# nipponjo/tts-arabic-pytorch

Hardware: AMD Instinct MI355X
Metric: audio samples/sec (FastPitch+HiFi-GAN, synthetic 64-phoneme inputs) (higher is better)
Workload: dtype f32

## Files before the change

tts-arabic-pytorch_amd/csrc/api.hip:

```cpp
#include <cerrno>
#include <cstdio>
#include <cstdlib>
#include <cstring>
#include <algorithm>
#include <atomic>
#include <mutex>
#include <string>
#include <vector>

#include "kernels.hpp"

namespace ttsamd {

static thread_local std::string g_err;

void set_error(const char* fmt, ...) {
    char buf[1024];
    va_list ap;
    va_start(ap, fmt);
    vsnprintf(buf, sizeof(buf), fmt, ap);
    va_end(ap);
    g_err = buf;
}

// ... 905 lines not shown
    float* wino = nullptr;
    if (default_precision() == 0 && convt_wino_packable(cin, cout, u) && opt_int(OPT_CONVT_WINO, 1) != 0) {
        wino = packed + 2 * n;
        const int64_t nw = (int64_t)(6 * cin + 1) * u * cout;
        hipLaunchKernelGGL(pack_convt_wino_kernel, dim3((unsigned)((nw + 255) / 256)), dim3(256), 0, s, w, bias, cin, cout, u, wino);
        TTS_CHECK_HIP(hipGetLastError());
    }
    ConvParams p;
    std::memset(&p, 0, sizeof(p));
    p.batch = batch;
    p.lens_in = lens; p.lens_out = lens;
    prof_begin(s, 2.0 * cout * cin * 2 * u);
    const int32_t rc = launch_upsampler(p, x, packed, planes, bias, y, cin, cout, u, 2 * u, lin, 1, in_slope, opt_int(OPT_CONVT, 1) != 0, s, wino,
                                        wino ? wino + (int64_t)6 * cin * u * cout : nullptr);
    prof_end(s);
    return rc;
}

int64_t ttsamd_resblock_pair_packed_floats(int32_t channels, int32_t k, int32_t variant) {
    if (channels < 1 || k < 1) return 0;
    const int64_t n = 2 * (int64_t)channels * k * channels;
    const int nwino = (variant == 4 ? 1 : (variant == 5 ? 2 : 0));
    if (variant == 6) return n + ((k == 3 || k == 7 || k == 11) ? 2 * (int64_t)channels * wino4_groups(k) * channels : 0);
    return n + ((k == 3 || k == 7 || k == 11) ? nwino * (int64_t)channels * wino2_groups(k) * channels : 0);
}

int32_t ttsamd_resblock_pair(const float* x, float* y, const float* w1, const float* b1, const float* w2, const float* b2,
                             int32_t channels, int32_t k, int32_t dil, const int64_t* lens, int32_t len_mul, int32_t L,
                             int32_t batch, int32_t mode, float div, float slope, int32_t variant, float* packed, int64_t packed_floats,
                             void* stream) {
    TTS_REQUIRE(x && y && w1 && b1 && w2 && b2 && packed && channels % 32 == 0 && k >= 1 && batch >= 1 && L >= 1 && len_mul >= 1 &&
                mode >= 0 && mode <= 2, "resblock_pair: bad argument");
    TTS_REQUIRE(packed_floats >= ttsamd_resblock_pair_packed_floats(channels, k, variant),
                "resblock_pair: `packed` holds %lld floats, variant %d at C = %d, k = %d needs %lld (ttsamd_resblock_pair_packed_floats)",
                (long long)packed_floats, variant, channels, k, (long long)ttsamd_resblock_pair_packed_floats(channels, k, variant));
    hipStream_t s = (hipStream_t)stream;
    const int64_t n = (int64_t)channels * k * channels;
    for (int i = 0; i < 2; ++i) {
        hipLaunchKernelGGL(pack_conv_weight_kernel, dim3((unsigned)((n + 255) / 256)), dim3(256), 0, s, i == 0 ? w1 : w2, channels,
                           channels, k, channels, packed + i * n);
        TTS_CHECK_HIP(hipGetLastError());
    }
    const double fl = 2.0 * (2.0 * channels * channels * k);
    int32_t rc;
    prof_begin(s, fl);
    if (variant == 1) {
// ... 4 lines not shown
            TTS_REQUIRE((k == 3 || k == 7 || k == 11) && (channels <= 64 || (variant == 5 && channels == 128)),
                        "resblock_pair: variants 4 / 5 are built for C = 32 / 64 (5: and 128), k = 3 / 7 / 11");
            const int64_t nw = (int64_t)channels * wino2_groups(k) * channels;
            for (int i = 0; i < (variant == 5 ? 2 : 1); ++i) {
                float* wino = packed + 2 * n + i * nw;
                hipLaunchKernelGGL(pack_wino2_weight_kernel, dim3((unsigned)((nw + 255) / 256)), dim3(256), 0, s, i == 0 ? w2 : w1, channels,
                                   channels, k, channels, wino);
                TTS_CHECK_HIP(hipGetLastError());
                (i == 0 ? w2w : w1w) = wino;
            }
        }
        rc = launch_fused_pair2(channels, x, y, packed, b1, packed + n, b2, k, dil, lens, len_mul, L, batch, mode, div, slope,
                                variant == 3 ? 1 : 2, s, w2w, w1w);
    } else if (variant == 6) {
        TTS_REQUIRE(channels == 32 && (k == 3 || k == 7 || k == 11), "resblock_pair: variant 6 is built for C = 32, k = 3 / 7 / 11");
        const int64_t nw4 = (int64_t)channels * wino4_groups(k) * channels;
        for (int i = 0; i < 2; ++i) {
            hipLaunchKernelGGL(pack_wino4_weight_kernel, dim3((unsigned)((nw4 + 255) / 256)), dim3(256), 0, s, i == 0 ? w1 : w2, channels,
                               channels, k, channels, packed + 2 * n + i * nw4);
            TTS_CHECK_HIP(hipGetLastError());
        }
        rc = launch_fused_pair4(channels, x, y, packed + 2 * n, b1, packed + 2 * n + nw4, b2, k, dil, lens, len_mul, L, batch, mode, div,
                                slope, s);
    } else if (variant == -1) {
        rc = 0;
    } else {
        set_error("resblock_pair: variant %d (1: first generation, 2 / 3: second generation with 256- / 128-column blocks, 4 / 5: 256 columns + Winograd phase B / both phases, 6: C = 32 with both phases on Winograd F(4,3))", variant);
        rc = TTSAMD_EINVAL;
    }
    prof_end(s);
    return rc;
}

int64_t ttsamd_resblock2_packed_floats(int32_t channels, int32_t k, int32_t variant) {
    if (channels < 1 || k < 1 || (variant != 1 && variant != 2)) return 0;
    return 2 * (int64_t)channels * k * channels;
}

int32_t ttsamd_resblock2(const float* x, float* y, const float* w1, const float* b1, const float* w2, const float* b2, int32_t channels,
                         int32_t k, int32_t dil1, int32_t dil2, const int64_t* lens, int32_t len_mul, int32_t L, int32_t batch, int32_t mode,
                         float div, float slope, int32_t variant, float* packed, int64_t packed_floats, void* stream) {
    TTS_REQUIRE(x && y && w1 && b1 && w2 && b2 && packed && channels % 32 == 0 && channels >= 32 && k >= 1 && batch >= 1 && L >= 1 &&
                len_mul >= 1 && mode >= 0 && mode <= 2 && x != y, "resblock2: bad argument");
    TTS_REQUIRE(variant == 1 || variant == 2, "resblock2: variant %d (1: two single-conv launches, 2: both convs in one launch)", variant);
    TTS_REQUIRE(packed_floats >= ttsamd_resblock2_packed_floats(channels, k, variant),
                "resblock2: `packed` holds %lld floats, C = %d, k = %d needs %lld (ttsamd_resblock2_packed_floats)", (long long)packed_floats,
                channels, k, (long long)ttsamd_resblock2_packed_floats(channels, k, variant));
    if (variant == 1) {
        TTS_REQUIRE(resblock2_conv_supported(channels, k, dil1, L, x, y) && resblock2_conv_supported(channels, k, dil2, L, x, y),
                    "resblock2: variant 1 does not cover C = %d, k = %d, dilations %d / %d (C = 32 / 64 / 128, k = 3 / 5 / 7 / 11, "
// ... 80 lines not shown
```

tts-arabic-pytorch_amd/csrc/common.hpp:

```cpp
#pragma once
#include <hip/hip_runtime.h>
#include <stdint.h>
#include <atomic>
#include <cstdarg>
#include <cstdio>
#include <cstdlib>
#include <string>

#include "../../include/ttsamd.h"

namespace ttsamd {

void set_error(const char* fmt, ...);

#define TTS_CHECK_HIP(expr)                                                         \
    do {                                                                            \
        hipError_t e_ = (expr);                                                     \
        if (e_ != hipSuccess) {                                                     \
            ttsamd::set_error("%s failed: %s (%s:%d)", #expr, hipGetErrorString(e_), \
                              __FILE__, __LINE__);                                  \
            return TTSAMD_EHIP;                                                     \
        }                                                                           \
    } while (0)

// ... 13 lines not shown

inline int64_t align_up(int64_t x, int64_t a) { return (x + a - 1) / a * a; }

inline hipError_t lds_opt_in(const void* fn, int bytes, std::atomic<uint64_t>& done) {
    int dev = 0;
    hipError_t e = hipGetDevice(&dev);
    if (e != hipSuccess) return e;
    if (dev >= 0 && dev < 64 && ((done.load(std::memory_order_acquire) >> dev) & 1)) return hipSuccess;
    e = hipFuncSetAttribute(fn, hipFuncAttributeMaxDynamicSharedMemorySize, bytes);
    if (e == hipSuccess && dev >= 0 && dev < 64) done.fetch_or(1ull << dev, std::memory_order_release);
    return e;
}

#define TTS_OPTIONS(X)                                                                                     \
    X(HIFIGAN_STREAMS, 0, 0, 1)    \
    X(WINO, 0, 0, 1)                                              \
    X(WINO2, 0, 0, 31)             \
    X(WINO4, 0, 0, 127)            \
    X(FUSED_PAIR, 0, 0, 1)                   \
    X(FUSED2, 0, 0, 1)                                           \
    X(FUSED2_MASK, 1, 0, 0x1ff)               \
    X(FUSED2_MASK_N1, 1, 0, 0x1ff)          \
    X(FUSED2_WB, 0, 0, 2)                     \
    X(PAIR4, 0, 0, 1)              \
    X(CONVT, 0, 0, 1)                              \
    X(CONVT_WINO, 0, 0, 2)         \
    X(BFO, 0, 0, 1)                \
    X(BFO_CHAIN, 0, 0, 1)                           \
    X(BFO_CHAIN7, 0, 0, 1)                                 \
    X(BFO_FF, 0, 0, 1)                              \
    X(BFO_SPLITK, 0, 0, 1)                                              \
    X(BFO_SMALL_TILES, 0, 0, 1)            \
    X(BF16_ATTN, 0, 0, 1)                                         \
    X(BF16_PACKED_T, 0, 0, 1)                   \
    X(ATT_RA, 0, 1, 4)                             \
    X(ATT_SPLIT, 0, 0, 1)                      \
    X(XCD_W, 0, 0, 1)                            \
    X(XCD_WMAX_KB, 0, 0, 1 << 20)     \
    X(DEEP_SPLITK, 0, 0, 1)        \
    X(TACO_PERSISTENT, 0, 0, 2)    \
    X(TACO_SEG, 0, 8, 1 << 20)     \
    X(RESBLOCK2_PAIR, 1, 0, 0x3f)
enum Opt : int {
#define TTS_OPT_ENUM(name, kind, lo, hi) OPT_##name,
    TTS_OPTIONS(TTS_OPT_ENUM)
#undef TTS_OPT_ENUM
    OPT_COUNT
// ... 68 lines not shown
void note_conv_launch(int32_t route, int32_t ksplit);
void last_conv_launch(int32_t* route, int32_t* ksplit);
bool convt_supported(const ConvParams& p);
int32_t launch_convt(const ConvParams& p, hipStream_t stream);
int32_t launch_upsampler(ConvParams& p, const float* x, const float* w, const void* w_bf16, const float* bias, float* y, int cin, int cout,
                         int u, int kt, int L, int len_mul, float in_slope, bool convt_ok, hipStream_t stream, const float* w_wino = nullptr,
                         const float* bias_wino = nullptr);
bool convt_wino_packable(int cin, int cout, int u);
void pack_convt_wino_weight(const float* w, const float* bias, int cin, int cout, int u, float* out_w, float* out_bias);
bool convt_wino_supported(const ConvParams& p, const float* w_wino, const float* bias_wino);
int32_t launch_convt_wino(const ConvParams& p, const float* w_wino, const float* bias_wino, hipStream_t stream);
bool fused_pair_supported(int32_t channels, int32_t k, int32_t dil, int32_t L, const float* x, const float* y);
int32_t launch_fused_pair(int32_t channels, const float* x, float* y, const float* w1, const float* b1, const float* w2,
                          const float* b2, int32_t k, int32_t dil, const int64_t* lens, int32_t len_mul, int32_t L, int32_t batch,
                          int32_t mode, float div, float slope, hipStream_t stream);
bool fused_pair2_supported(int32_t channels, int32_t k, int32_t dil, int32_t L, const float* x, const float* y, int32_t ntw);
int32_t launch_fused_pair2(int32_t channels, const float* x, float* y, const float* w1, const float* b1, const float* w2,
                           const float* b2, int32_t k, int32_t dil, const int64_t* lens, int32_t len_mul, int32_t L, int32_t batch,
                           int32_t mode, float div, float slope, int32_t ntw, hipStream_t stream, const float* w2_wino = nullptr,
                           const float* w1_wino = nullptr);
bool fused_pair4_supported(int32_t channels, int32_t k, int32_t dil, int32_t L, const float* x, const float* y);
int32_t launch_fused_pair4(int32_t channels, const float* x, float* y, const float* w1_wino4, const float* b1, const float* w2_wino4,
                           const float* b2, int32_t k, int32_t dil, const int64_t* lens, int32_t len_mul, int32_t L, int32_t batch,
                           int32_t mode, float div, float slope, hipStream_t stream);
bool resblock2_conv_supported(int32_t channels, int32_t k, int32_t dil, int32_t L, const float* x, const float* y);
int32_t launch_resblock2_conv(int32_t channels, const float* x, float* y, const float* w, const float* b, int32_t k, int32_t dil,
                              const int64_t* lens, int32_t len_mul, int32_t L, int32_t batch, int32_t mode, float div, float slope,
                              hipStream_t stream);
bool resblock2_pair_supported(int32_t channels, int32_t k, int32_t d1, int32_t d2, int32_t L, const float* x, const float* y);
int32_t launch_resblock2_pair(int32_t channels, const float* x, float* y, const float* w1, const float* b1, const float* w2,
                              const float* b2, int32_t k, int32_t d1, int32_t d2, const int64_t* lens, int32_t len_mul, int32_t L,
                              int32_t batch, int32_t mode, float div, float slope, hipStream_t stream);
int wino_route(const ConvParams& p);
int32_t launch_wino(const ConvParams& p, hipStream_t stream);
void pack_wino_weight(const float* w, int cout, int cin, float* out);
int wino2_groups(int k);
int wino2_block_outputs(int coutp, int dil);
int32_t launch_wino2(const ConvParams& p, hipStream_t stream);
void pack_wino2_weight(const float* w, int cout, int cin, int k, float* out);
int wino4_groups(int k);
int wino44_groups(int k);
constexpr int kWino4Default = 127;
bool wino44_wanted(const ConvParams& p);
int wino4_block_outputs(int dil);
int wino4_ksplit(const ConvParams& p);
int32_t launch_splitk_reduce(const ConvParams& q, hipStream_t stream);
int32_t launch_wino4(const ConvParams& p, hipStream_t stream);
// ... 48 lines not shown
```

tts-arabic-pytorch_amd/csrc/hifigan.hip:

```cpp
#include <cmath>
#include <cstring>
#include <cstdlib>
#include <map>
#include <mutex>
#include <string>
#include <vector>

#include "kernels.hpp"
#include "bfo.hpp"

namespace ttsamd {

constexpr unsigned kFused2Mask = 0x00F;
constexpr int kPair4MinK = 7;
constexpr unsigned kFused2MaskN1 = 0x000;
constexpr int64_t kFused2SmallColumns = 2 * 256 * 252;

constexpr unsigned kResblock2PairMask = 0x00;

static bool resblock2_pair_choice(unsigned mask, int32_t channels, int32_t k, int32_t d1, int32_t d2, int32_t L, const float* x,
                                  const float* y) {
    const int ci = channels == 32 ? 0 : (channels == 64 ? 1 : -1);
    const int ki = k == 3 ? 0 : (k == 5 ? 1 : (k == 7 ? 2 : -1));
    if (ci < 0 || ki < 0 || !(mask & (1u << (3 * ci + ki)))) return false;
    return resblock2_pair_supported(channels, k, d1, d2, L, x, y);
}

struct ConvW {
    int64_t w_off = 0, b_off = 0;
    int64_t w16_off = 0, w_n = 0;
    BfoWeightOffs wo;
    int64_t ww44_off = -1;
    int64_t ww4_off = -1;
    int64_t wct_off = -1, bct_off = -1;
    int64_t ww_off = -1;
    int cin = 0, cout = 0, k = 0;
};
// ... 9 lines not shown
    int hop = 1;
    bool rb2 = false;
    int64_t max_cl = 0;
    bool bfo_ok = false;
    mutable std::mutex mu;
    mutable hipStream_t side[2] = {nullptr, nullptr};
    mutable hipEvent_t ev_fork = nullptr, ev_done[3] = {nullptr, nullptr, nullptr};
};

static bool use_branch_streams(const HifiGan* h, int32_t B, int32_t T) {
    if (h->cfg.n_kernels != 3) return false;
    const int64_t streams = opt_int(OPT_HIFIGAN_STREAMS, -1);
    if (streams >= 0) return streams == 1;
    if (default_precision() == 1 && h->bfo_ok) {
        if (opt_int(OPT_BFO, 1) != 0) return (int64_t)B * T >= 8192;
    }
    return true;
}

struct Fused2Switches {
    bool on = true, mask_forced = false;
    bool wino_b = true, wino_a = true;
    bool pair4 = true;
    unsigned mask = kFused2Mask, mask_n1 = kFused2MaskN1;
};
static Fused2Switches read_fused2_switches() {
    Fused2Switches sw;
    sw.on = opt_int(OPT_FUSED2, 1) != 0;
    const int64_t m = opt_int(OPT_FUSED2_MASK, -1);
    sw.mask_forced = m >= 0;
    if (sw.mask_forced) sw.mask = (unsigned)m;
    sw.mask_n1 = (unsigned)opt_int(OPT_FUSED2_MASK_N1, kFused2MaskN1);
    const int64_t wb = opt_int(OPT_FUSED2_WB, 2);
    sw.wino_b = wb != 0;
    sw.wino_a = wb == 2;
    sw.pair4 = opt_int(OPT_PAIR4, 1) != 0;
    return sw;
}

static int fused2_choice(const Fused2Switches& sw, int32_t channels, int32_t k, int32_t dil, int32_t L, const float* x, const float* y,
                         int64_t columns) {
    if (!sw.on) return 0;
    const int ci = channels == 32 ? 0 : (channels == 64 ? 1 : (channels == 128 ? 2 : -1));
    const int ki = k == 3 ? 0 : (k == 7 ? 1 : (k == 11 ? 2 : -1));
    if (ci < 0 || ki < 0) return 0;
    const unsigned bit = 1u << (3 * ci + ki);
    const bool small = columns < (int64_t)kFused2SmallColumns && !sw.mask_forced;
    if (small) return 0;
    if (!(sw.mask & bit)) return 0;
    int ntw = (sw.mask_n1 & bit) ? 1 : 2;
    if (!fused_pair2_supported(channels, k, dil, L, x, y, ntw)) {
        ntw = 3 - ntw;
        if (!fused_pair2_supported(channels, k, dil, L, x, y, ntw)) return 0;
    }
    return ntw;
}

using TensorMap = std::map<std::string, const ttsamd_tensor*>;

// ... 66 lines not shown
    TTS_TRY(folded_weight(tm, base, 3, w, shp));
    TTS_REQUIRE(shp[0] == cout && shp[1] == cin && shp[2] == k, "hifigan: '%s' has shape [%lld,%lld,%lld], expected [%d,%d,%d]",
                base.c_str(), (long long)shp[0], (long long)shp[1], (long long)shp[2], cout, cin, k);
    cw.cin = cin; cw.cout = cout; cw.k = k;
    cw.w_off = (int64_t)blob.size();
    blob.resize(blob.size() + (size_t)cin * k * cout_padded(cout));
    pack_conv_weight(w.data(), cout, cin, k, blob.data() + cw.w_off);
    if (direct_only) {
        blob.resize(align_up((int64_t)blob.size(), 64));
        return get_bias(tm, base, cout, blob, cw.b_off);
    }
    add_bf16(blob, blob16, cw, (int64_t)cin * k * cout_padded(cout));
    if ((k == 3 || k == 7 || k == 11) && cin % 8 == 0 && cout % 32 == 0) {
        blob.resize(align_up((int64_t)blob.size(), 64));
        cw.ww_off = (int64_t)blob.size();
        blob.resize(blob.size() + (size_t)cin * wino2_groups(k) * cout_padded(cout));
        pack_wino2_weight(w.data(), cout, cin, k, blob.data() + cw.ww_off);
        if (cout >= 64 || (cout == 32 && cin == 32 && k >= kPair4MinK)) {
            blob.resize(align_up((int64_t)blob.size(), 64));
            cw.ww4_off = (int64_t)blob.size();
            blob.resize(blob.size() + (size_t)cin * wino4_groups(k) * cout_padded(cout));
            pack_wino4_weight(w.data(), cout, cin, k, blob.data() + cw.ww4_off);
        }
        if (cout >= 64 && wino44_groups(k) != 0) {
            blob.resize(align_up((int64_t)blob.size(), 64));
            cw.ww44_off = (int64_t)blob.size();
            blob.resize(blob.size() + (size_t)cin * wino44_groups(k) * cout_padded(cout));
            pack_wino44_weight(w.data(), cout, cin, k, blob.data() + cw.ww44_off);
        }
    }
    if (cin % 8 == 0 && cout % 32 == 0) cw.wo = bfo_append_weights(w.data(), cout, cin, k, 1, blob16);
    blob.resize(align_up((int64_t)blob.size(), 64));
    return get_bias(tm, base, cout, blob, cw.b_off);
}

void hifigan_destroy(HifiGan* h);

__global__ void hifigan_touch_kernel() {}

int32_t hifigan_create(const ttsamd_tensor* weights, int32_t n, const ttsamd_hifigan_cfg* cfg, HifiGan** out) {
    TTS_REQUIRE(weights && cfg && out, "hifigan_create: null argument");
    TTS_REQUIRE(cfg->n_ups >= 1 && cfg->n_ups <= 8 && cfg->n_kernels >= 1 && cfg->n_kernels <= 8 &&
                cfg->n_dilations >= 1 && cfg->n_dilations <= 8, "hifigan_create: bad config counts");
    const int rb = cfg->resblock == 0 ? 1 : cfg->resblock;
    TTS_REQUIRE(rb == 1 || rb == 2, "hifigan_create: resblock %d (1 = ResBlock1, 2 = ResBlock2)", cfg->resblock);
    TTS_REQUIRE(rb == 1 || cfg->n_dilations >= 2, "hifigan_create: a ResBlock2 takes two dilations per kernel size, %d given",
                cfg->n_dilations);
// ... 203 lines not shown
    } join{false, bs[1], bs[2]};
    const auto fail = [&](int32_t rc) { join.on = multi && rc != 0; return rc; };

    ConvParams p;
    std::memset(&p, 0, sizeof(p));
    p.batch = B;
    p.lens_in = lens; p.lens_out = lens;
    p.n_phase = 1; p.div = 1.f;
    p.splitk_ws = splitks[0]; p.splitk_floats = kSplitKFloats;
    const bool pack_t = default_precision() == 1 && opt_int(OPT_BF16_PACKED_T, 1) != 0;
    const Fused2Switches f2sw = read_fused2_switches();
    const bool fused_ok = default_precision() == 0 && opt_int(OPT_FUSED_PAIR, 1) != 0;
    const bool convt_ok = opt_int(OPT_CONVT, 1) != 0;
    const unsigned rb2_mask = (unsigned)opt_int(OPT_RESBLOCK2_PAIR, kResblock2PairMask);
    bool in_section = false;
    int pack_io = 0;
    auto conv = [&](const ConvW& cw, const float* x, hipStream_t st, float* y, const float* res, int L, int mul,
                    int dil, float slope, int mode, float div) -> int32_t {
        p.x = x; p.x_bs = (int64_t)cw.cin * L; p.x_cs = L;
        p.w = h->dev + cw.w_off; p.bias = h->dev + cw.b_off;
        p.w_bf16 = h->dev16 + cw.w16_off; p.precision = default_precision();
        p.w_wino = cw.ww_off >= 0 ? h->dev + cw.ww_off : nullptr;
        p.w_wino4 = (cw.ww4_off >= 0 && cw.cout >= 64) ? h->dev + cw.ww4_off : nullptr;
        p.w_wino44 = cw.ww44_off >= 0 ? h->dev + cw.ww44_off : nullptr;
        p.y = y; p.y_bs = (int64_t)cw.cout * L; p.y_cs = L; p.y_ts = 1;
        p.res = res; p.r_bs = (int64_t)cw.cout * L; p.r_cs = L;
        p.len_in_mul = mul; p.len_out_mul = mul; p.Lin = L; p.Nout = L;
        p.Cin = cw.cin; p.Cout = cw.cout; p.CoutP = cout_padded(cw.cout); p.K = cw.k;
        p.dil = dil; p.pad = (cw.k * dil - dil) / 2;
        p.n_phase = 1; p.phase_p = 0;
        p.in_slope = slope; p.relu_out = 0; p.mode = mode; p.div = div;
        p.x_packed = (pack_io & 1) ? 1 : 0; p.y_packed = (pack_io & 2) ? 1 : 0; p.pack_slope = 0.1f;
        if (in_section) prof_add(2.0 * cw.cout * cw.cin * cw.k * mul);
        else prof_begin(st, 2.0 * cw.cout * cw.cin * cw.k * mul);
        const int32_t rc = launch_conv(p, st);
        if (!in_section) prof_end(st);
        return rc;
    };

#define HG_TRY(expr) do { int32_t rc_ = (expr); if (rc_ != 0) return fail(rc_); } while (0)
#define HG_CHECK_HIP(expr) do { hipError_t e_ = (expr); if (e_ != hipSuccess) { set_error("%s failed: %s (%s:%d)", #expr, hipGetErrorString(e_), __FILE__, __LINE__); return fail(TTSAMD_EHIP); } } while (0)
    const int prec = default_precision();
    if ((prec == 1 || prec == 2) && h->bfo_ok && opt_int(OPT_BFO, 1) != 0) {
        const BfoMode& M = bfo_mode(prec);
        const uint16_t* W16 = h->dev16;
        void *curo = cur, *upso = ups_out;
        HG_TRY(M.pack(mel, B, cfg.num_mels, T, 1.f, mel_o, s));
// ... 155 lines not shown
                                            0.1f, st);
                if (!in_section) prof_end(st);
                HG_TRY(rc2);
            }
            if (multi) HG_CHECK_HIP(hipEventRecord(h->ev_done[j], st));
        }
        for (int j = 0; !h->rb2 && j < cfg.n_kernels; ++j) {
            hipStream_t st = bs[j % 3];
            float *Tb = Tbs[j % 3], *R = Rs[j % 3];
            p.splitk_ws = splitks[j % 3];
            if (multi && j > 0) HG_CHECK_HIP(hipStreamWaitEvent(st, h->ev_fork, 0));
            const float* src = ups_out;
            for (int m = 0; m < cfg.n_dilations; ++m) {
                const int li = (i * cfg.n_kernels + j) * cfg.n_dilations + m;
                const int d = cfg.resblock_dilations[j][m];
                {
                    const bool last = m + 1 == cfg.n_dilations;
                    float* dst = last ? cur : (src == R ? Tb : R);
                    const ConvW &w1 = h->c1[li], &w2 = h->c2[li];
                    const bool square = w1.cin == w1.cout && w2.cin == w1.cin && w2.cout == w1.cin && w1.k == w2.k;
                    const int ntw2 = (fused_ok && square) ? fused2_choice(f2sw, w1.cin, w1.k, d, L, src, dst, (int64_t)B * L) : 0;
                    const bool f43 = ntw2 == 2 && f2sw.pair4 && f2sw.wino_a && w1.k >= kPair4MinK && w1.ww4_off >= 0 && w2.ww4_off >= 0 &&
                                     fused_pair4_supported(w1.cin, w1.k, d, L, src, dst);
                    if (ntw2 != 0 || (fused_ok && square && fused_pair_supported(w1.cin, w1.k, d, L, src, dst))) {
                        const int mode = !last ? 0 : (cfg.n_kernels == 1 ? 0 : (j == 0 ? 0 : (j + 1 < cfg.n_kernels ? 1 : 2)));
                        if (multi && last && j > 0) HG_CHECK_HIP(hipStreamWaitEvent(st, h->ev_done[j - 1], 0));
                        const double fl = 2.0 * (2.0 * w1.cin * w1.cin * w1.k) * mul;
                        if (in_section) prof_add(fl); else prof_begin(st, fl);
                        const int32_t frc = f43
                            ? launch_fused_pair4(w1.cin, src, dst, h->dev + w1.ww4_off, h->dev + w1.b_off, h->dev + w2.ww4_off,
                                                 h->dev + w2.b_off, w1.k, d, lens, mul, L, B, mode, (float)cfg.n_kernels, 0.1f, st)
                            : ntw2 != 0
                            ? launch_fused_pair2(w1.cin, src, dst, h->dev + w1.w_off, h->dev + w1.b_off, h->dev + w2.w_off,
                                                 h->dev + w2.b_off, w1.k, d, lens, mul, L, B, mode, (float)cfg.n_kernels, 0.1f, ntw2, st,
                                                 (f2sw.wino_b && w2.ww_off >= 0) ? h->dev + w2.ww_off : nullptr,
                                                 (f2sw.wino_a && w1.ww_off >= 0) ? h->dev + w1.ww_off : nullptr)
                            : launch_fused_pair(w1.cin, src, dst, h->dev + w1.w_off, h->dev + w1.b_off, h->dev + w2.w_off,
                                                h->dev + w2.b_off, w1.k, d, lens, mul, L, B, mode, (float)cfg.n_kernels, 0.1f, st);
                        if (!in_section) prof_end(st);
                        HG_TRY(frc);
                        if (multi && last) HG_CHECK_HIP(hipEventRecord(h->ev_done[j], st));
                        src = dst;
                        continue;
                    }
                }
                pack_io = pack_t ? 2 : 0;
                HG_TRY(conv(h->c1[li], src, st, Tb, nullptr, L, mul, d, 0.1f, 0, 1.f));
                pack_io = pack_t ? 1 : 0;
                if (m + 1 < cfg.n_dilations) {
                    HG_TRY(conv(h->c2[li], Tb, st, R, src, L, mul, 1, 0.1f, 0, 1.f));
                    pack_io = 0;
                    src = R;
// ... 34 lines not shown
```

tts-arabic-pytorch_amd/csrc/resblock_pair4.hip:

```cpp
#include <algorithm>
#include <cstring>

#include "conv_mfma_common.hpp"
#include "bfo.hpp"

namespace ttsamd {

struct FusedPair4Params {
    const float* x;
    float* y;
    const float4* w1;
    const float4* w2;
    const float* b1;
    const float* b2;
    const int64_t* lens;
    int32_t len_mul, L, dil, batch;
    int32_t mode;
    float div, slope;
    int32_t compact;
};

template <int K>
struct Pair4Geo {
    static constexpr int C = 32, NOCT = C / 8;
    static constexpr int H = (K - 1) / 2;
    static constexpr int NSF = K == 3 ? 1 : (K == 7 ? 2 : 4);
    static constexpr int NTAP = K == 7 ? 4 : 0;
    static constexpr int NG = K == 3 ? 6 : (K == 7 ? 16 : 23);
    static constexpr int NGQ = (NG + 1) & ~1;
    static constexpr int NPL = K == 7 ? 8 : 6;
    static constexpr int NPOS = K + 3;
    static constexpr int NBU = NSF + (NTAP ? 1 : 0);
    static constexpr int PF = 4;
    static constexpr int UO = (NGQ % PF == 0) ? 1 : 2;
    static_assert((UO * NGQ) % PF == 0 && NOCT % UO == 0, "queue slots");
    static constexpr int NQ = 128;
    static constexpr int WQ = 145;
    static constexpr int ROW = 4 * WQ;
    static constexpr int LDS_BYTES = 2 * NOCT * ROW * 16;
    static_assert(LDS_BYTES <= 80 * 1024, "two blocks per CU");
    __host__ __device__ static constexpr int nqa(int d) { return (4 * NQ / (4 * d)) * d; }
    __host__ __device__ static constexpr int ts(int d) { return (4 * nqa(d) - 2 * H) & ~3; }
    __host__ __device__ static constexpr int nvec(int d) { return (3 + 4 * nqa(d) + (K - 1) * d + 3) / 4; }
    static_assert(nvec(1) <= WQ && nvec(3) <= WQ && nvec(5) <= WQ, "window fits a sub-row");
    static_assert((4 * NQ - 4 + NPOS - 1) / 4 < WQ, "phase B reads stay inside a sub-row");
    __host__ __device__ static constexpr int bpos(int u) { return u < NSF ? 3 * u : 3 * NSF; }
    __host__ __device__ static constexpr int bnum(int u) { return u < NSF ? (3 * u + 5 < NPOS ? 6 : 5) : 4; }
};

__device__ __forceinline__ float p4_lrelu(const float v, const float slope) {
    return __builtin_amdgcn_fmed3f(v, v * slope, __builtin_inff());
}

typedef float p4_f4 __attribute__((ext_vector_type(4)));

__device__ __forceinline__ p4_f4 p4v(const float4 a) { return p4_f4{a.x, a.y, a.z, a.w}; }

template <int K>
__device__ __forceinline__ void p4_conv(f32x16 (&acc)[Pair4Geo<K>::NPL], float4 (&aq)[Pair4Geo<K>::PF], const float4* xs,
                                        const int (&eo)[Pair4Geo<K>::NPOS], const float4* __restrict__ wl,
                                        const float4* __restrict__ wnext) {
    using G = Pair4Geo<K>;
    constexpr int C = G::C, NOCT = G::NOCT, NSF = G::NSF, NGQ = G::NGQ, PF = G::PF, UO = G::UO, NBU = G::NBU, ROW = G::ROW;
    constexpr int NGT = NOCT * NGQ;
    float4 xq[2][6];
#pragma unroll
    for (int m = 0; m < G::bnum(0); ++m) xq[0][m] = xs[eo[G::bpos(0) + m]];
#pragma unroll 1
    for (int ob = 0; ob < NOCT; ob += UO) {
#pragma unroll
        for (int bi = 0; bi < UO * NBU; ++bi) {
            const int ol = bi / NBU, u = bi % NBU, cur = bi & 1, nxt = cur ^ 1;
            const int o = ob + ol;
            {
                const int un = (u + 1) % NBU;
                const int on = min(u + 1 < NBU ? o : o + 1, NOCT - 1);
                const float4* xn = xs + on * 2 * ROW;
#pragma unroll
                for (int m = 0; m < G::bnum(un); ++m) xq[nxt][m] = xn[eo[G::bpos(un) + m]];
            }
            p4_f4 x[6];
#pragma unroll
            for (int m = 0; m < G::bnum(u); ++m) x[m] = p4v(xq[cur][m]);
            const bool sub = u < NSF;
            const int ng = sub ? 6 : 4;
#pragma unroll
            for (int i = 0; i < ng; ++i) {
                const int g = sub ? 6 * u + i : 6 * NSF + i;
                const int gb = ol * NGQ + g;
                const int slot = gb % PF;
                const float4 a4 = aq[slot];
                {
                    const int gn = o * NGQ + g + PF;
                    const float4* __restrict__ src = gn < NGT ? wl + gn * 2 * C : wnext + (gn - NGT) * 2 * C;
                    aq[slot] = *src;
                }
                if (g >= G::NG) continue;
                p4_f4 v;
                int plane;
                if (sub) {
                    plane = i;
                    if (i == 0) v = 4.f * x[0] + (x[4] - 5.f * x[2]);
                    else if (i == 1) v = (x[4] - 4.f * x[2]) + (x[3] - 4.f * x[1]);
                    else if (i == 2) v = (x[4] - 4.f * x[2]) - (x[3] - 4.f * x[1]);
                    else if (i == 3) v = (x[4] - x[2]) + 2.f * (x[3] - x[1]);
                    else if (i == 4) v = (x[4] - x[2]) - 2.f * (x[3] - x[1]);
                    else v = 4.f * x[1] + (x[5] - 5.f * x[3]);
                } else {
                    plane = i == 0 ? 0 : (i == 1 ? 6 : (i == 2 ? 7 : 5));
                    v = x[i];
                }
                __builtin_amdgcn_sched_barrier(0);
                const float av[4] = {a4.x, a4.y, a4.z, a4.w};
#pragma unroll
                for (int pq = 0; pq < 4; ++pq) acc[plane] = __builtin_amdgcn_mfma_f32_32x32x2f32(av[pq], v[pq], acc[plane], 0, 0, 0);
            }
        }
        if ((UO * NBU) & 1) {
#pragma unroll
            for (int m = 0; m < 6; ++m) xq[0][m] = xq[1][m];
        }
    }
}

template <int NPL>
__device__ __forceinline__ void p4_out(const f32x16 (&acc)[NPL], const int r, float (&y)[4]) {
    const float s12 = acc[1][r] + acc[2][r], d12 = acc[1][r] - acc[2][r];
    const float s34 = acc[3][r] + acc[4][r], d34 = acc[3][r] - acc[4][r];
    y[0] = acc[0][r] + s12 + s34;
    y[1] = d12 + 2.f * d34;
    y[2] = s12 + 4.f * s34;
    y[3] = d12 + 8.f * d34 + acc[5][r];
    if constexpr (NPL == 8) {
        y[1] += acc[6][r];
        y[2] += acc[7][r];
    }
}

template <int K>
__global__ __launch_bounds__(256, 2) void resblock_pair4(const FusedPair4Params p) {
    using G = Pair4Geo<K>;
    constexpr int C = G::C, NOCT = G::NOCT, H = G::H, NPL = G::NPL, NPOS = G::NPOS, PF = G::PF, WQ = G::WQ, ROW = G::ROW;
    extern __shared__ __attribute__((aligned(16))) float4 smem4[];
    const int dil = p.dil, L = p.L;
    const int TS = G::ts(dil);
    const int tid = threadIdx.x, lane = tid & 63, wid = tid >> 6;
    const int kk = lane >> 5, l31 = lane & 31;
    int b = blockIdx.z;
    int q0 = blockIdx.x * TS;
    if (p.compact) {
        int tile = 0;
        if (!live_tile(p.lens, p.len_mul, L, TS, p.batch, blockIdx.z * gridDim.x + blockIdx.x, b, tile)) return;
        b = __builtin_amdgcn_readfirstlane(b);
        q0 = __builtin_amdgcn_readfirstlane(tile) * TS;
    }
    int len = L;
    if (p.lens) len = min(len, (int)p.lens[b] * p.len_mul);
    if (q0 >= len) return;
    const float slope = p.slope;
    const float* __restrict__ xb = p.x + (int64_t)b * C * L;
    float4* Xs = smem4;

    const float4* __restrict__ wl1 = p.w1 + kk * C + l31;
    const float4* __restrict__ wl2 = p.w2 + kk * C + l31;
// ... 31 lines not shown
                    Xs[row * ROW + j * WQ + vi] = make_float4(p4_lrelu(vv[0][j], slope), p4_lrelu(vv[1][j], slope),
                                                              p4_lrelu(vv[2][j], slope), p4_lrelu(vv[3][j], slope));
            }
        }
    }
    __syncthreads();

    const int jw = wid * 32 + l31;
    const int nqa = G::nqa(dil);
    const int pa = min(jw, nqa - 1);
    const int na = dil == 1 ? 4 * pa : (pa / dil) * 4 * dil + pa % dil;
    f32x16 acc[NPL];
#pragma unroll
    for (int g = 0; g < NPL; ++g)
#pragma unroll
        for (int r = 0; r < 16; ++r) acc[g][r] = 0.f;
    {
        int eo[NPOS];
#pragma unroll
        for (int m = 0; m < NPOS; ++m) {
            const int c = off + na + m * dil;
            eo[m] = (c & 3) * WQ + (c >> 2);
        }
        p4_conv<K>(acc, aq, Xs + kk * ROW, eo, wl1, wl2);
    }
    __syncthreads();
    if (jw < nqa) {
        float bias[16];
#pragma unroll
        for (int r = 0; r < 16; ++r) bias[r] = p.b1[(r & 3) + 8 * (r >> 2) + 4 * kk];
        float y[16][4];
#pragma unroll
        for (int r = 0; r < 16; ++r) p4_out<NPL>(acc, r, y[r]);
#pragma unroll
        for (int h = 0; h < 4; ++h) {
            const int c = na + h * dil;
            const int pos = q0 - H + c;
            const bool live = pos >= 0 && pos < len;
            const int ent = (c & 3) * WQ + (c >> 2);
#pragma unroll
            for (int oc = 0; oc < 4; ++oc)
#pragma unroll
                for (int k2 = 0; k2 < 2; ++k2) {
                    const int r = 4 * oc + k2;
                    const float v0 = p4_lrelu(y[r][h] + bias[r], slope), v1 = p4_lrelu(y[r + 2][h] + bias[r + 2], slope);
                    const float2 w2v = live ? make_float2(v0, v1) : make_float2(0.f, 0.f);
                    *reinterpret_cast<float2*>(reinterpret_cast<float*>(Xs + (2 * oc + k2) * ROW + ent) + 2 * kk) = w2v;
                }
        }
    }
    __syncthreads();

#pragma unroll
    for (int g = 0; g < NPL; ++g)
#pragma unroll
        for (int r = 0; r < 16; ++r) acc[g][r] = 0.f;
    {
        int eo[NPOS];
#pragma unroll
        for (int m = 0; m < NPOS; ++m) eo[m] = (m & 3) * WQ + jw + (m >> 2);
        p4_conv<K>(acc, aq, Xs + kk * ROW, eo, wl2, wl2);
    }

    const int n = 4 * jw, q = q0 + n;
    if (n >= TS || q >= len) return;
    const bool full = q + 3 < len;
    float* __restrict__ yb = p.y + (int64_t)b * C * L;
    const int mode = p.mode;
    const float div = p.div;
#pragma unroll
    for (int r = 0; r < 16; ++r) {
        const int ch = (r & 3) + 8 * (r >> 2) + 4 * kk;
        float v[4];
        p4_out<NPL>(acc, r, v);
        const float bs = p.b2[ch];
        const float* xp = xb + (int64_t)ch * L + q;
        float* yp = yb + (int64_t)ch * L + q;
        float xr[4] = {0.f, 0.f, 0.f, 0.f}, yr[4] = {0.f, 0.f, 0.f, 0.f};
        if (full) {
            const float4 t = *reinterpret_cast<const float4*>(xp);
            xr[0] = t.x; xr[1] = t.y; xr[2] = t.z; xr[3] = t.w;
            if (mode != 0) { const float4 s = *reinterpret_cast<const float4*>(yp); yr[0] = s.x; yr[1] = s.y; yr[2] = s.z; yr[3] = s.w; }
        } else {
#pragma unroll
            for (int e = 0; e < 4; ++e)
                if (q + e < len) {
                    xr[e] = xp[e];
                    if (mode != 0) yr[e] = yp[e];
                }
        }
#pragma unroll
        for (int e = 0; e < 4; ++e) {
            float t = v[e] + bs + xr[e];
            if (mode == 1) t = yr[e] + t;
            else if (mode == 2) t = (yr[e] + t) / div;
            v[e] = t;
        }
        if (full) {
            *reinterpret_cast<float4*>(yp) = make_float4(v[0], v[1], v[2], v[3]);
        } else {
#pragma unroll
            for (int e = 0; e < 4; ++e)
                if (q + e < len) yp[e] = v[e];
        }
    }
}

template <int K>
static int32_t launch_pair4_k(const FusedPair4Params& p, hipStream_t stream) {
    using G = Pair4Geo<K>;
    static std::atomic<uint64_t> lds_done{0};
    TTS_CHECK_HIP(lds_opt_in((const void*)resblock_pair4<K>, G::LDS_BYTES, lds_done));
    const int ts = G::ts(p.dil);
    dim3 grid((p.L + ts - 1) / ts, 1, p.batch);
    hipLaunchKernelGGL(resblock_pair4<K>, grid, dim3(256), G::LDS_BYTES, stream, p);
    TTS_CHECK_HIP(hipGetLastError());
    return 0;
}

bool fused_pair4_supported(int32_t channels, int32_t k, int32_t dil, int32_t L, const float* x, const float* y) {
    if (channels != 32 || !(k == 3 || k == 7 || k == 11) || !(dil == 1 || dil == 3 || dil == 5)) return false;
    if (L < 4 || (L & 3) != 0 || ((((uintptr_t)x) | ((uintptr_t)y)) & 15) != 0 || x == y) return false;
    return (int64_t)channels * L * 4 < ((int64_t)1 << 31);
}

int32_t launch_fused_pair4(int32_t channels, const float* x, float* y, const float* w1_wino4, const float* b1, const float* w2_wino4,
                           const float* b2, int32_t k, int32_t dil, const int64_t* lens, int32_t len_mul, int32_t L, int32_t batch,
                           int32_t mode, float div, float slope, hipStream_t stream) {
    TTS_REQUIRE(fused_pair4_supported(channels, k, dil, L, x, y),
                "fused ResBlock pair (F(4,3)): unsupported geometry (C=%d, k=%d, dil=%d, L=%d)", channels, k, dil, L);
    TTS_REQUIRE(w1_wino4 && w2_wino4 && b1 && b2, "fused ResBlock pair (F(4,3)): null weights");
    TTS_REQUIRE(slope > 0.f && slope <= 1.f, "fused ResBlock pair (F(4,3)): leaky-relu slope %g outside (0, 1]", (double)slope);
    TTS_REQUIRE(mode >= 0 && mode <= 2 && (mode != 2 || div != 0.f), "fused ResBlock pair (F(4,3)): bad mode / div");
    conv_log("fused_pair4", k, channels, channels, L, batch, 1, mode, len_mul, lens != nullptr, 1);
    FusedPair4Params p;
    std::memset(&p, 0, sizeof(p));
    p.x = x; p.y = y;
    p.w1 = reinterpret_cast<const float4*>(w1_wino4); p.w2 = reinterpret_cast<const float4*>(w2_wino4);
    p.b1 = b1; p.b2 = b2; p.lens = lens; p.len_mul = len_mul; p.L = L; p.dil = dil; p.batch = batch;
    p.mode = mode; p.div = div; p.slope = slope;
    p.compact = compact_order(lens, batch) ? 1 : 0;
    if (k == 3) return launch_pair4_k<3>(p, stream);
    if (k == 7) return launch_pair4_k<7>(p, stream);
    return launch_pair4_k<11>(p, stream);
}

}
```

Before: 77.09 million.

## Add seven-point Winograd group variant for C=32 fused ResBlock pair kernels

Adds a seven-point grouping of the F(4,3)-style Winograd transform for the fused C=32 ResBlock pair kernel at k = 7 and 11, with new input-transform arithmetic, an extra output plane folded in with scaled weights, and packing of wino44 weights for 32-channel convs. It becomes the default path when PAIR4 is 1 for both kernel sizes. The intent is to cut the number of transformed groups and per-group MFMA work compared with the six-point layout. In exchange it adds register pressure from the extra saved intermediates, a different queue-unroll factor, and more host weight packing.

```diff
diff --git a/tts-arabic-pytorch_amd/csrc/api.hip b/tts-arabic-pytorch_amd/csrc/api.hip
--- a/tts-arabic-pytorch_amd/csrc/api.hip
+++ b/tts-arabic-pytorch_amd/csrc/api.hip
@@ -951,6 +951,7 @@
     const int64_t n = 2 * (int64_t)channels * k * channels;
     const int nwino = (variant == 4 ? 1 : (variant == 5 ? 2 : 0));
     if (variant == 6) return n + ((k == 3 || k == 7 || k == 11) ? 2 * (int64_t)channels * wino4_groups(k) * channels : 0);
+    if (variant == 7) return n + 2 * (int64_t)channels * wino44_groups(k) * channels;
     return n + ((k == 3 || k == 7 || k == 11) ? nwino * (int64_t)channels * wino2_groups(k) * channels : 0);
 }
 
@@ -1001,10 +1002,20 @@
         }
         rc = launch_fused_pair4(channels, x, y, packed + 2 * n, b1, packed + 2 * n + nw4, b2, k, dil, lens, len_mul, L, batch, mode, div,
                                 slope, s);
+    } else if (variant == 7) {
+        TTS_REQUIRE(channels == 32 && (k == 7 || k == 11), "resblock_pair: variant 7 is built for C = 32, k = 7 / 11");
+        const int64_t nw44 = (int64_t)channels * wino44_groups(k) * channels;
+        for (int i = 0; i < 2; ++i) {
+            hipLaunchKernelGGL(pack_wino44_weight_kernel, dim3((unsigned)((nw44 + 255) / 256)), dim3(256), 0, s, i == 0 ? w1 : w2, channels,
+                               channels, k, channels, packed + 2 * n + i * nw44);
+            TTS_CHECK_HIP(hipGetLastError());
+        }
+        rc = launch_fused_pair4(channels, x, y, packed + 2 * n, b1, packed + 2 * n + nw44, b2, k, dil, lens, len_mul, L, batch, mode, div,
+                                slope, s, 7);
     } else if (variant == -1) {
         rc = 0;
     } else {
-        set_error("resblock_pair: variant %d (1: first generation, 2 / 3: second generation with 256- / 128-column blocks, 4 / 5: 256 columns + Winograd phase B / both phases, 6: C = 32 with both phases on Winograd F(4,3))", variant);
+        set_error("resblock_pair: variant %d (1: first generation, 2 / 3: second generation with 256- / 128-column blocks, 4 / 5: 256 columns + Winograd phase B / both phases, 6: C = 32 with both phases on Winograd F(4,3), 7: ... on its seven-point groups, k = 7 / 11)", variant);
         rc = TTSAMD_EINVAL;
     }
     prof_end(s);
diff --git a/tts-arabic-pytorch_amd/csrc/common.hpp b/tts-arabic-pytorch_amd/csrc/common.hpp
--- a/tts-arabic-pytorch_amd/csrc/common.hpp
+++ b/tts-arabic-pytorch_amd/csrc/common.hpp
@@ -59,7 +59,7 @@
     X(FUSED2_MASK, 1, 0, 0x1ff)               \
     X(FUSED2_MASK_N1, 1, 0, 0x1ff)          \
     X(FUSED2_WB, 0, 0, 2)                     \
-    X(PAIR4, 0, 0, 1)              \
+    X(PAIR4, 0, 0, 2)              \
     X(CONVT, 0, 0, 1)                              \
     X(CONVT_WINO, 0, 0, 2)         \
     X(BFO, 0, 0, 1)                \
@@ -174,7 +174,7 @@
 bool fused_pair4_supported(int32_t channels, int32_t k, int32_t dil, int32_t L, const float* x, const float* y);
 int32_t launch_fused_pair4(int32_t channels, const float* x, float* y, const float* w1_wino4, const float* b1, const float* w2_wino4,
                            const float* b2, int32_t k, int32_t dil, const int64_t* lens, int32_t len_mul, int32_t L, int32_t batch,
-                           int32_t mode, float div, float slope, hipStream_t stream);
+                           int32_t mode, float div, float slope, hipStream_t stream, int32_t points = 6);
 bool resblock2_conv_supported(int32_t channels, int32_t k, int32_t dil, int32_t L, const float* x, const float* y);
 int32_t launch_resblock2_conv(int32_t channels, const float* x, float* y, const float* w, const float* b, int32_t k, int32_t dil,
                               const int64_t* lens, int32_t len_mul, int32_t L, int32_t batch, int32_t mode, float div, float slope,
diff --git a/tts-arabic-pytorch_amd/csrc/hifigan.hip b/tts-arabic-pytorch_amd/csrc/hifigan.hip
--- a/tts-arabic-pytorch_amd/csrc/hifigan.hip
+++ b/tts-arabic-pytorch_amd/csrc/hifigan.hip
@@ -13,6 +13,7 @@
 
 constexpr unsigned kFused2Mask = 0x00F;
 constexpr int kPair4MinK = 7;
+constexpr unsigned kPair44Mask = 0x3;
 constexpr unsigned kFused2MaskN1 = 0x000;
 constexpr int64_t kFused2SmallColumns = 2 * 256 * 252;
 
@@ -68,6 +69,7 @@
     bool on = true, mask_forced = false;
     bool wino_b = true, wino_a = true;
     bool pair4 = true;
+    bool pair44 = true;
     unsigned mask = kFused2Mask, mask_n1 = kFused2MaskN1;
 };
 static Fused2Switches read_fused2_switches() {
@@ -80,7 +82,9 @@
     const int64_t wb = opt_int(OPT_FUSED2_WB, 2);
     sw.wino_b = wb != 0;
     sw.wino_a = wb == 2;
-    sw.pair4 = opt_int(OPT_PAIR4, 1) != 0;
+    const int64_t p4 = opt_int(OPT_PAIR4, 1);
+    sw.pair4 = p4 != 0;
+    sw.pair44 = p4 == 1;
     return sw;
 }
 
@@ -193,7 +197,7 @@
             blob.resize(blob.size() + (size_t)cin * wino4_groups(k) * cout_padded(cout));
             pack_wino4_weight(w.data(), cout, cin, k, blob.data() + cw.ww4_off);
         }
-        if (cout >= 64 && wino44_groups(k) != 0) {
+        if ((cout >= 64 || (cout == 32 && cin == 32 && k >= kPair4MinK)) && wino44_groups(k) != 0) {
             blob.resize(align_up((int64_t)blob.size(), 64));
             cw.ww44_off = (int64_t)blob.size();
             blob.resize(blob.size() + (size_t)cin * wino44_groups(k) * cout_padded(cout));
@@ -443,7 +447,7 @@
         p.w_bf16 = h->dev16 + cw.w16_off; p.precision = default_precision();
         p.w_wino = cw.ww_off >= 0 ? h->dev + cw.ww_off : nullptr;
         p.w_wino4 = (cw.ww4_off >= 0 && cw.cout >= 64) ? h->dev + cw.ww4_off : nullptr;
-        p.w_wino44 = cw.ww44_off >= 0 ? h->dev + cw.ww44_off : nullptr;
+        p.w_wino44 = (cw.ww44_off >= 0 && cw.cout >= 64) ? h->dev + cw.ww44_off : nullptr;
         p.y = y; p.y_bs = (int64_t)cw.cout * L; p.y_cs = L; p.y_ts = 1;
         p.res = res; p.r_bs = (int64_t)cw.cout * L; p.r_cs = L;
         p.len_in_mul = mul; p.len_out_mul = mul; p.Lin = L; p.Nout = L;
@@ -645,12 +649,17 @@
                     const int ntw2 = (fused_ok && square) ? fused2_choice(f2sw, w1.cin, w1.k, d, L, src, dst, (int64_t)B * L) : 0;
                     const bool f43 = ntw2 == 2 && f2sw.pair4 && f2sw.wino_a && w1.k >= kPair4MinK && w1.ww4_off >= 0 && w2.ww4_off >= 0 &&
                                      fused_pair4_supported(w1.cin, w1.k, d, L, src, dst);
+                    const bool f44 = f43 && f2sw.pair44 && (kPair44Mask & (w1.k == 7 ? 1u : (w1.k == 11 ? 2u : 0u))) != 0 &&
+                                     w1.ww44_off >= 0 && w2.ww44_off >= 0;
                     if (ntw2 != 0 || (fused_ok && square && fused_pair_supported(w1.cin, w1.k, d, L, src, dst))) {
                         const int mode = !last ? 0 : (cfg.n_kernels == 1 ? 0 : (j == 0 ? 0 : (j + 1 < cfg.n_kernels ? 1 : 2)));
                         if (multi && last && j > 0) HG_CHECK_HIP(hipStreamWaitEvent(st, h->ev_done[j - 1], 0));
                         const double fl = 2.0 * (2.0 * w1.cin * w1.cin * w1.k) * mul;
                         if (in_section) prof_add(fl); else prof_begin(st, fl);
-                        const int32_t frc = f43
+                        const int32_t frc = f44
+                            ? launch_fused_pair4(w1.cin, src, dst, h->dev + w1.ww44_off, h->dev + w1.b_off, h->dev + w2.ww44_off,
+                                                 h->dev + w2.b_off, w1.k, d, lens, mul, L, B, mode, (float)cfg.n_kernels, 0.1f, st, 7)
+                            : f43
                             ? launch_fused_pair4(w1.cin, src, dst, h->dev + w1.ww4_off, h->dev + w1.b_off, h->dev + w2.ww4_off,
                                                  h->dev + w2.b_off, w1.k, d, lens, mul, L, B, mode, (float)cfg.n_kernels, 0.1f, st)
                             : ntw2 != 0
diff --git a/tts-arabic-pytorch_amd/csrc/resblock_pair4.hip b/tts-arabic-pytorch_amd/csrc/resblock_pair4.hip
--- a/tts-arabic-pytorch_amd/csrc/resblock_pair4.hip
+++ b/tts-arabic-pytorch_amd/csrc/resblock_pair4.hip
@@ -20,19 +20,22 @@
     int32_t compact;
 };
 
-template <int K>
+template <int K, int PT_ = 6>
 struct Pair4Geo {
+    static constexpr bool PT7 = PT_ == 7;
+    static_assert(PT_ == 6 || (PT7 && (K == 7 || K == 11)), "seven-point groups: k = 7 / 11");
     static constexpr int C = 32, NOCT = C / 8;
     static constexpr int H = (K - 1) / 2;
-    static constexpr int NSF = K == 3 ? 1 : (K == 7 ? 2 : 4);
-    static constexpr int NTAP = K == 7 ? 4 : 0;
-    static constexpr int NG = K == 3 ? 6 : (K == 7 ? 16 : 23);
-    static constexpr int NGQ = (NG + 1) & ~1;
-    static constexpr int NPL = K == 7 ? 8 : 6;
+    static constexpr int NSF = PT7 ? (K + 3) / 4 : (K == 3 ? 1 : (K == 7 ? 2 : 4));
+    static constexpr int NTAP = (!PT7 && K == 7) ? 4 : 0;
+    static constexpr int NG = PT7 ? 7 * NSF - 1 : (K == 3 ? 6 : (K == 7 ? 16 : 23));
+    static constexpr int NGQ = PT7 ? NG : (NG + 1) & ~1;
+    static constexpr int NPL = PT7 ? 7 : (K == 7 ? 8 : 6);
     static constexpr int NPOS = K + 3;
     static constexpr int NBU = NSF + (NTAP ? 1 : 0);
+    static constexpr int NX = PT7 ? 7 : 6;
     static constexpr int PF = 4;
-    static constexpr int UO = (NGQ % PF == 0) ? 1 : 2;
+    static constexpr int UO = (NGQ % PF == 0) ? 1 : ((2 * NGQ) % PF == 0 ? 2 : 4);
     static_assert((UO * NGQ) % PF == 0 && NOCT % UO == 0, "queue slots");
     static constexpr int NQ = 128;
     static constexpr int WQ = 145;
@@ -44,8 +47,9 @@
     __host__ __device__ static constexpr int nvec(int d) { return (3 + 4 * nqa(d) + (K - 1) * d + 3) / 4; }
     static_assert(nvec(1) <= WQ && nvec(3) <= WQ && nvec(5) <= WQ, "window fits a sub-row");
     static_assert((4 * NQ - 4 + NPOS - 1) / 4 < WQ, "phase B reads stay inside a sub-row");
-    __host__ __device__ static constexpr int bpos(int u) { return u < NSF ? 3 * u : 3 * NSF; }
-    __host__ __device__ static constexpr int bnum(int u) { return u < NSF ? (3 * u + 5 < NPOS ? 6 : 5) : 4; }
+    __host__ __device__ static constexpr int bpos(int u) { return PT7 ? 4 * u : (u < NSF ? 3 * u : 3 * NSF); }
+    __host__ __device__ static constexpr int bnum(int u) { return PT7 ? (4 * u + 3 < K ? 7 : 6) : (u < NSF ? (3 * u + 5 < NPOS ? 6 : 5) : 4); }
+    static_assert(bpos(NBU - 1) + bnum(NBU - 1) <= NPOS, "the last bundle ends inside the window");
 };
 
 __device__ __forceinline__ float p4_lrelu(const float v, const float slope) {
@@ -56,14 +60,13 @@
 
 __device__ __forceinline__ p4_f4 p4v(const float4 a) { return p4_f4{a.x, a.y, a.z, a.w}; }
 
-template <int K>
-__device__ __forceinline__ void p4_conv(f32x16 (&acc)[Pair4Geo<K>::NPL], float4 (&aq)[Pair4Geo<K>::PF], const float4* xs,
-                                        const int (&eo)[Pair4Geo<K>::NPOS], const float4* __restrict__ wl,
-                                        const float4* __restrict__ wnext) {
-    using G = Pair4Geo<K>;
-    constexpr int C = G::C, NOCT = G::NOCT, NSF = G::NSF, NGQ = G::NGQ, PF = G::PF, UO = G::UO, NBU = G::NBU, ROW = G::ROW;
+template <int K, int PT_, typename G = Pair4Geo<K, PT_>>
+__device__ __forceinline__ void p4_conv(f32x16 (&acc)[G::NPL], float4 (&aq)[G::PF], const float4* xs, const int (&eo)[G::NPOS],
+                                        const float4* __restrict__ wl, const float4* __restrict__ wnext) {
+    constexpr int C = G::C, NOCT = G::NOCT, NSF = G::NSF, NGQ = G::NGQ, PF = G::PF, UO = G::UO, NBU = G::NBU, ROW = G::ROW, NX = G::NX;
+    constexpr bool PT7 = G::PT7;
     constexpr int NGT = NOCT * NGQ;
-    float4 xq[2][6];
+    float4 xq[2][NX];
 #pragma unroll
     for (int m = 0; m < G::bnum(0); ++m) xq[0][m] = xs[eo[G::bpos(0) + m]];
 #pragma unroll 1
@@ -79,14 +82,15 @@
 #pragma unroll
                 for (int m = 0; m < G::bnum(un); ++m) xq[nxt][m] = xn[eo[G::bpos(un) + m]];
             }
-            p4_f4 x[6];
+            p4_f4 x[NX];
 #pragma unroll
             for (int m = 0; m < G::bnum(u); ++m) x[m] = p4v(xq[cur][m]);
             const bool sub = u < NSF;
-            const int ng = sub ? 6 : 4;
+            const int ng = PT7 ? G::bnum(u) : (sub ? 6 : 4);
+            p4_f4 f1, f3, f4, e1, e2, h1, h2;
 #pragma unroll
             for (int i = 0; i < ng; ++i) {
-                const int g = sub ? 6 * u + i : 6 * NSF + i;
+                const int g = PT7 ? 7 * u + i : (sub ? 6 * u + i : 6 * NSF + i);
                 const int gb = ol * NGQ + g;
                 const int slot = gb % PF;
                 const float4 a4 = aq[slot];
@@ -98,7 +102,31 @@
                 if (g >= G::NG) continue;
                 p4_f4 v;
                 int plane;
-                if (sub) {
+                if constexpr (PT7) {
+                    plane = i;
+                    if (i == 0) {
+                        const p4_f4 f0 = x[2] - 4.f * x[0], f2 = x[4] - 4.f * x[2];
+                        f1 = x[3] - 4.f * x[1];
+                        f3 = x[5] - 4.f * x[3];
+                        if (ng == 7) f4 = x[6] - 4.f * x[4];
+                        const p4_f4 e0 = f0 - 2.f * f1;
+                        e2 = f2 - 2.f * f3;
+                        e1 = f1 - 2.f * f2;
+                        v = e2 - e0;
+                    } else if (i == 1) v = e1 + e2;
+                    else if (i == 2) v = e1 - e2;
+                    else if (i == 3) {
+                        const p4_f4 d1 = x[1] - x[3], d2 = x[2] - x[4], d3 = x[3] - x[5];
+                        h1 = d1 - 2.f * d2;
+                        h2 = d2 - 2.f * d3;
+                        v = 2.f * h1 + h2;
+                    } else if (i == 4) v = 2.f * h1 - h2;
+                    else if (i == 5) v = f3 - f1;
+                    else {
+                        const p4_f4 e3 = f3 - 2.f * f4;
+                        v = e1 - e3;
+                    }
+                } else if (sub) {
                     plane = i;
                     if (i == 0) v = 4.f * x[0] + (x[4] - 5.f * x[2]);
                     else if (i == 1) v = (x[4] - 4.f * x[2]) + (x[3] - 4.f * x[1]);
@@ -118,28 +146,33 @@
         }
         if ((UO * NBU) & 1) {
 #pragma unroll
-            for (int m = 0; m < 6; ++m) xq[0][m] = xq[1][m];
-        }
-    }
-}
-
-template <int NPL>
+            for (int m = 0; m < NX; ++m) xq[0][m] = xq[1][m];
+        }
+    }
+}
+
+template <int PT_, int NPL>
 __device__ __forceinline__ void p4_out(const f32x16 (&acc)[NPL], const int r, float (&y)[4]) {
     const float s12 = acc[1][r] + acc[2][r], d12 = acc[1][r] - acc[2][r];
     const float s34 = acc[3][r] + acc[4][r], d34 = acc[3][r] - acc[4][r];
     y[0] = acc[0][r] + s12 + s34;
     y[1] = d12 + 2.f * d34;
     y[2] = s12 + 4.f * s34;
-    y[3] = d12 + 8.f * d34 + acc[5][r];
-    if constexpr (NPL == 8) {
+    y[3] = d12 + 8.f * d34 + acc[PT_ == 7 ? 6 : 5][r];
+    if constexpr (PT_ == 7) {
+        y[0] += acc[5][r];
+        y[1] += 0.5f * acc[5][r];
+        y[2] += 0.25f * acc[5][r];
+        y[3] += 0.125f * acc[5][r];
+    } else if constexpr (NPL == 8) {
         y[1] += acc[6][r];
         y[2] += acc[7][r];
     }
 }
 
-template <int K>
+template <int K, int PT_ = 6>
 __global__ __launch_bounds__(256, 2) void resblock_pair4(const FusedPair4Params p) {
-    using G = Pair4Geo<K>;
+    using G = Pair4Geo<K, PT_>;
     constexpr int C = G::C, NOCT = G::NOCT, H = G::H, NPL = G::NPL, NPOS = G::NPOS, PF = G::PF, WQ = G::WQ, ROW = G::ROW;
     extern __shared__ __attribute__((aligned(16))) float4 smem4[];
     const int dil = p.dil, L = p.L;
@@ -217,7 +250,7 @@
             const int c = off + na + m * dil;
             eo[m] = (c & 3) * WQ + (c >> 2);
         }
-        p4_conv<K>(acc, aq, Xs + kk * ROW, eo, wl1, wl2);
+        p4_conv<K, PT_>(acc, aq, Xs + kk * ROW, eo, wl1, wl2);
     }
     __syncthreads();
     if (jw < nqa) {
@@ -226,7 +259,7 @@
         for (int r = 0; r < 16; ++r) bias[r] = p.b1[(r & 3) + 8 * (r >> 2) + 4 * kk];
         float y[16][4];
 #pragma unroll
-        for (int r = 0; r < 16; ++r) p4_out<NPL>(acc, r, y[r]);
+        for (int r = 0; r < 16; ++r) p4_out<PT_, NPL>(acc, r, y[r]);
 #pragma unroll
         for (int h = 0; h < 4; ++h) {
             const int c = na + h * dil;
@@ -254,7 +287,7 @@
         int eo[NPOS];
 #pragma unroll
         for (int m = 0; m < NPOS; ++m) eo[m] = (m & 3) * WQ + jw + (m >> 2);
-        p4_conv<K>(acc, aq, Xs + kk * ROW, eo, wl2, wl2);
+        p4_conv<K, PT_>(acc, aq, Xs + kk * ROW, eo, wl2, wl2);
     }
 
     const int n = 4 * jw, q = q0 + n;
@@ -267,7 +300,7 @@
     for (int r = 0; r < 16; ++r) {
         const int ch = (r & 3) + 8 * (r >> 2) + 4 * kk;
         float v[4];
-        p4_out<NPL>(acc, r, v);
+        p4_out<PT_, NPL>(acc, r, v);
         const float bs = p.b2[ch];
         const float* xp = xb + (int64_t)ch * L + q;
         float* yp = yb + (int64_t)ch * L + q;
@@ -301,14 +334,14 @@
     }
 }
 
-template <int K>
+template <int K, int PT_ = 6>
 static int32_t launch_pair4_k(const FusedPair4Params& p, hipStream_t stream) {
-    using G = Pair4Geo<K>;
+    using G = Pair4Geo<K, PT_>;
     static std::atomic<uint64_t> lds_done{0};
-    TTS_CHECK_HIP(lds_opt_in((const void*)resblock_pair4<K>, G::LDS_BYTES, lds_done));
+    TTS_CHECK_HIP(lds_opt_in((const void*)resblock_pair4<K, PT_>, G::LDS_BYTES, lds_done));
     const int ts = G::ts(p.dil);
     dim3 grid((p.L + ts - 1) / ts, 1, p.batch);
-    hipLaunchKernelGGL(resblock_pair4<K>, grid, dim3(256), G::LDS_BYTES, stream, p);
+    hipLaunchKernelGGL((resblock_pair4<K, PT_>), grid, dim3(256), G::LDS_BYTES, stream, p);
     TTS_CHECK_HIP(hipGetLastError());
     return 0;
 }
@@ -321,13 +354,15 @@
 
 int32_t launch_fused_pair4(int32_t channels, const float* x, float* y, const float* w1_wino4, const float* b1, const float* w2_wino4,
                            const float* b2, int32_t k, int32_t dil, const int64_t* lens, int32_t len_mul, int32_t L, int32_t batch,
-                           int32_t mode, float div, float slope, hipStream_t stream) {
+                           int32_t mode, float div, float slope, hipStream_t stream, int32_t points) {
     TTS_REQUIRE(fused_pair4_supported(channels, k, dil, L, x, y),
                 "fused ResBlock pair (F(4,3)): unsupported geometry (C=%d, k=%d, dil=%d, L=%d)", channels, k, dil, L);
+    TTS_REQUIRE(points == 6 || (points == 7 && (k == 7 || k == 11)),
+                "fused ResBlock pair (F(4,3)): %d-point groups at k = %d (six-point: k = 3 / 7 / 11, seven-point: k = 7 / 11)", points, k);
     TTS_REQUIRE(w1_wino4 && w2_wino4 && b1 && b2, "fused ResBlock pair (F(4,3)): null weights");
     TTS_REQUIRE(slope > 0.f && slope <= 1.f, "fused ResBlock pair (F(4,3)): leaky-relu slope %g outside (0, 1]", (double)slope);
     TTS_REQUIRE(mode >= 0 && mode <= 2 && (mode != 2 || div != 0.f), "fused ResBlock pair (F(4,3)): bad mode / div");
-    conv_log("fused_pair4", k, channels, channels, L, batch, 1, mode, len_mul, lens != nullptr, 1);
+    conv_log(points == 7 ? "fused_pair44" : "fused_pair4", k, channels, channels, L, batch, 1, mode, len_mul, lens != nullptr, 1);
     FusedPair4Params p;
     std::memset(&p, 0, sizeof(p));
     p.x = x; p.y = y;
@@ -335,6 +370,7 @@
     p.b1 = b1; p.b2 = b2; p.lens = lens; p.len_mul = len_mul; p.L = L; p.dil = dil; p.batch = batch;
     p.mode = mode; p.div = div; p.slope = slope;
     p.compact = compact_order(lens, batch) ? 1 : 0;
+    if (points == 7) return k == 7 ? launch_pair4_k<7, 7>(p, stream) : launch_pair4_k<11, 7>(p, stream);
     if (k == 3) return launch_pair4_k<3>(p, stream);
     if (k == 7) return launch_pair4_k<7>(p, stream);
     return launch_pair4_k<11>(p, stream);
```

New measurement: 77.95 million, median of 6. 1.01x the previous value.
